# ivanacollg/MPC_CollisionAvoidance

Measured on AMD Instinct MI355X. Metric: batched SQP-RTI solves/sec (USV, N=40 horizon, 10 obstacles), higher is better.
Workload: dtype f64

## Files before the change

mpc_collisionavoidance_amd/csrc/gfx950/lanes.hpp:

```cpp
#pragma once
#include <hip/hip_runtime.h>

#define USV_DEV __device__ __forceinline__

namespace lanes {

constexpr int GROUP = 16;

USV_DEV int lane() { return (int)(threadIdx.x & 15u); }
USV_DEV long group_linear() { return (long)blockIdx.x * (long)(blockDim.x >> 4) + (long)(threadIdx.x >> 4); }

template <int CTRL>
USV_DEV double dpp_mov(double v)
{
    const long l = __builtin_bit_cast(long, v);
    const long r = __builtin_amdgcn_update_dpp(0L, l, CTRL, 0xf, 0xf, true);
    return __builtin_bit_cast(double, r);
}

template <int K>
USV_DEV double bcast(double v)
{
    static_assert(K >= 0 && K < 16, "lane index");
    return dpp_mov<0x150 + K>(v);
// ... 26 lines not shown
}
template <int K0, int K1, int K2>
USV_DEV void fma_bc3(double &c, double b0, double a0, double b1, double a1, double b2, double a2)
{
    asm(USV_DPP_HEAD "v_fmac_f64_dpp %0, %1, %2 row_newbcast:%7 row_mask:0xf bank_mask:0xf\n\t"
        "v_fmac_f64_dpp %0, %3, %4 row_newbcast:%8 row_mask:0xf bank_mask:0xf\n\t"
        "v_fmac_f64_dpp %0, %5, %6 row_newbcast:%9 row_mask:0xf bank_mask:0xf"
        : "+&v"(c) : "v"(b0), "v"(a0), "v"(b1), "v"(a1), "v"(b2), "v"(a2), "n"(K0), "n"(K1), "n"(K2));
}
template <int K0, int K1, int K2, int K3>
USV_DEV void fma_bc4(double &c, double b0, double a0, double b1, double a1, double b2, double a2, double b3, double a3)
{
    asm(USV_DPP_HEAD "v_fmac_f64_dpp %0, %1, %2 row_newbcast:%9 row_mask:0xf bank_mask:0xf\n\t"
        "v_fmac_f64_dpp %0, %3, %4 row_newbcast:%10 row_mask:0xf bank_mask:0xf\n\t"
        "v_fmac_f64_dpp %0, %5, %6 row_newbcast:%11 row_mask:0xf bank_mask:0xf\n\t"
        "v_fmac_f64_dpp %0, %7, %8 row_newbcast:%12 row_mask:0xf bank_mask:0xf"
        : "+&v"(c) : "v"(b0), "v"(a0), "v"(b1), "v"(a1), "v"(b2), "v"(a2), "v"(b3), "v"(a3), "n"(K0), "n"(K1), "n"(K2), "n"(K3));
}

USV_DEV void settle(double &v)
{
    asm volatile("s_nop 1" : "+v"(v));
}

USV_DEV double gather(double v, int src)
{
    const int addr = (int)((((unsigned)threadIdx.x & 48u) | ((unsigned)src & 15u)) << 2);
    const long l = __builtin_bit_cast(long, v);
    const int lo = __builtin_amdgcn_ds_bpermute(addr, (int)l);
    const int hi = __builtin_amdgcn_ds_bpermute(addr, (int)(l >> 32));
    return __builtin_bit_cast(double, ((long)(unsigned)lo) | ((long)hi << 32));
}

template <int N>
USV_DEV double ror(double v)
{
    static_assert(N >= 1 && N < 16, "rotation");
    return dpp_mov<0x120 + N>(v);
}

USV_DEV double gsum(double v)
{
    v += ror<8>(v);
    v += ror<4>(v);
    v += ror<2>(v);
    v += ror<1>(v);
    return v;
}
USV_DEV double vmax(double a, double b)
{
    double r;
    asm("v_max_f64 %0, %1, %2" : "=v"(r) : "v"(a), "v"(b));
    return r;
}
USV_DEV double vmax_abs(double a, double b)
{
    double r;
    asm("v_max_f64 %0, %1, |%2|" : "=v"(r) : "v"(a), "v"(b));
    return r;
}
USV_DEV double vmax_abs2(double a, double b)
{
    double r;
    asm("v_max_f64 %0, |%1|, |%2|" : "=v"(r) : "v"(a), "v"(b));
    return r;
}
USV_DEV double gmax(double v)
{
    v = vmax(v, ror<8>(v));
    v = vmax(v, ror<4>(v));
    v = vmax(v, ror<2>(v));
    v = vmax(v, ror<1>(v));
    return v;
}
USV_DEV double gmin(double v)
{
    v = fmin(v, ror<8>(v));
    v = fmin(v, ror<4>(v));
    v = fmin(v, ror<2>(v));
    v = fmin(v, ror<1>(v));
    return v;
}

USV_DEV int uniform(int v) { return __builtin_amdgcn_readfirstlane(v); }

USV_DEV void sched_fence() { __builtin_amdgcn_sched_barrier(0); }

USV_DEV void count_one(int *p) { atomicAdd(p, 1); }
USV_DEV int fetch_add(int *p) { return atomicAdd(p, 1); }

USV_DEV bool wave_any(bool p) { return __any((int)p) != 0; }

USV_DEV double frcp(double x)
{
    double r = __builtin_amdgcn_rcp(x);
    r = __builtin_fma(__builtin_fma(-x, r, 1.0), r, r);
    r = __builtin_fma(__builtin_fma(-x, r, 1.0), r, r);
    return r;
}
USV_DEV void frcp2(double a, double b, double &ia, double &ib)
{
    const double r = frcp(a * b);
    ia = r * b;
    ib = r * a;
}
USV_DEV double frsqrt(double x)
{
    double y = __builtin_amdgcn_rsq(x);
    y = __builtin_fma(0.5 * y, __builtin_fma(-x * y, y, 1.0), y);
    y = __builtin_fma(0.5 * y, __builtin_fma(-x * y, y, 1.0), y);
    return y;
}

USV_DEV void st_shared(double *p, double v)
{
    __hip_atomic_store(reinterpret_cast<unsigned long long *>(p), __builtin_bit_cast(unsigned long long, v), __ATOMIC_RELAXED, __HIP_MEMORY_SCOPE_AGENT);
}
// ... 119 lines not shown
```

mpc_collisionavoidance_amd/csrc/lin_order.hpp:

```cpp
#pragma once

#if defined(__HIPCC__) || defined(__CUDACC__)
#define USV_HD __host__ __device__ inline
#else
#define USV_HD inline
#endif

namespace usv {

struct LinItem {
    long g;
    int k;
};

USV_HD long lin_slot(long g, long B) { return g < B ? g : B - 1; }

USV_HD LinItem lin_item(long item, int N, long B, const int *perm_cur, const int *inv_next)
{
    const long q = item / (N + 1);
    LinItem it;
    it.k = (int)(item - q * (N + 1));
    it.g = q;
    if (q < B) {
        const long b = perm_cur ? (long)perm_cur[q] : q;
        it.g = inv_next ? (long)inv_next[b] : b;
    }
    return it;
}

}
```

mpc_collisionavoidance_amd/csrc/linearize.hpp:

```cpp
#pragma once
#include "lanes.hpp"
#include "lin_order.hpp"
#include "params.hpp"
#include "sfor.hpp"

namespace usv {

template <class M, class = void>
struct ModelCall {
    struct Pre {};
    USV_DEV static Pre prepare(const double *) { return {}; }
    USV_DEV static void fjvp(const Pre &, const double *x, const double *U, const double *s, const double *su, double *f, double *js)
    {
        M::fjvp(x, U, s, su, f, js);
    }
};
template <class M>
struct ModelCall<M, std::void_t<typename M::Pre>> {
    using Pre = typename M::Pre;
    USV_DEV static Pre prepare(const double *x) { return M::prepare(x); }
    USV_DEV static void fjvp(const Pre &p, const double *x, const double *U, const double *s, const double *su, double *f, double *js)
    {
        M::fjvp_pre(p, x, U, s, su, f, js);
    }
};

template <class M, int KCH, bool SOFT, bool MULTI = false, int MODE = 0>
struct Linearize {
    static constexpr int NX = M::NX, NU = M::NU, NZ = NX + NU;
    using WL = WsLayout<M, KCH, SOFT>;
    static constexpr bool SPEC = MODE == 1 || MODE == 3, FIXUP = MODE == 2 || MODE == 4;

    USV_DEV static void run(const DevPtrs &P, long gid)
    {
        const long Bp = lanes::uniform(P.spec->Bp);
        const int k = (int)(gid / Bp);
        run_at(P, k, gid - (long)k * Bp);
    }

    USV_DEV static void run_item(const DevPtrs &P, long item)
    {
        const LinItem it = lin_item(item, P.spec->N, (long)P.spec->B, P.perm_cur, P.inv_next);
        run_at(P, it.k, it.g);
    }

    USV_DEV static void run_marked(const DevPtrs &P, long g, int row)
    {
        const int N = lanes::uniform(P.spec->N);
        const long gi = lin_slot(g, (long)lanes::uniform(P.spec->B));
        const long b = P.perm ? (long)P.perm[gi] : gi;
        int any = 0;
        for (int w = 0; w < P.redo_words; w++) any |= P.redo[b * P.redo_words + w];
        if (any == 0) return;
        for (int k = row; k <= N; k += lanes::WAVE_ROWS) run_at(P, k, g);
    }

    USV_DEV static void run_at(const DevPtrs &P, const int k, const long g)
    {
// ... 12 lines not shown
            }
        }
        if constexpr (FIXUP) {
            if (((P.redo[b * P.redo_words + (k >> 5)] >> (k & 31)) & 1) == 0) return;
        }
        auto ld = [](const double *q) {
            if constexpr (SPEC) return lanes::ld_shared(q);
            else return *q;
        };
        double *tile = P.ws + (((long)k * Bp + g) * lanes::uniform(S.npt)) * LANES + lane;
        const bool xlane = lane >= NU && lane < NZ;

        double x[NX], U[NU > 0 ? NU : 1];
        const double *xk = P.x + ((long)b * (N + 1) + k) * NX;
        sfor<0, NX>([&](auto i) { x[i] = ld(xk + i); });
        if (k < N) {
            const double *uk = P.u + ((long)b * N + k) * NU;
            sfor<0, NU>([&](auto i) { U[i] = ld(uk + i); });
        } else {
            sfor<0, NU>([&](auto i) { U[i] = 0.0; });
        }

        {
            const double *Mrow = (k < N ? S.Mc : S.Me) + lane * LANES;
            const double *yr = (k < N) ? P.yref + ((long)b * N + k) * S.ny : P.yref_e + (long)b * S.ny_e;
            const int ny = (k < N) ? S.ny : S.ny_e;
            double acc = 0.0;
            for (int y = 0; y < ny; y++) acc = fma(-Mrow[y], yr[y], acc);
            tile[WL::P_GQ * LANES] = acc;
        }
        if (k == N) return;

        const int nsteps = MULTI ? S.sim_steps : 1;
        const double dt = S.dt / (double)nsteps;
        double s0[NX], f[NX], js[NX], xs[NX], ss[NX], xa[NX], sa[NX], su[NU > 0 ? NU : 1];
        sfor<0, NU>([&](auto l) { su[l] = (lane == l) ? 1.0 : 0.0; });
        sfor<0, NX>([&](auto i) { s0[i] = (lane == NU + i) ? 1.0 : 0.0; });
        using MC = ModelCall<M>;
        const typename MC::Pre pre = MC::prepare(x);
        for (int step = 0; step < nsteps; step++) {
            MC::fjvp(pre, x, U, s0, su, f, js);
            sfor<0, NX>([&](auto i) {
                xa[i] = f[i];
                sa[i] = js[i];
                xs[i] = fma(0.5 * dt, f[i], x[i]);
                ss[i] = fma(0.5 * dt, js[i], s0[i]);
            });
            MC::fjvp(pre, xs, U, ss, su, f, js);
            sfor<0, NX>([&](auto i) {
                xa[i] = fma(2.0, f[i], xa[i]);
                sa[i] = fma(2.0, js[i], sa[i]);
                xs[i] = fma(0.5 * dt, f[i], x[i]);
                ss[i] = fma(0.5 * dt, js[i], s0[i]);
            });
            MC::fjvp(pre, xs, U, ss, su, f, js);
            sfor<0, NX>([&](auto i) {
                xa[i] = fma(2.0, f[i], xa[i]);
                sa[i] = fma(2.0, js[i], sa[i]);
                xs[i] = fma(dt, f[i], x[i]);
                ss[i] = fma(dt, js[i], s0[i]);
            });
            MC::fjvp(pre, xs, U, ss, su, f, js);
            sfor<0, NX>([&](auto i) {
                x[i] = fma(dt / 6.0, xa[i] + f[i], x[i]);
                sa[i] = fma(dt / 6.0, sa[i] + js[i], s0[i]);
                if constexpr (MULTI) s0[i] = sa[i];
            });
        }
        const double *xn = P.x + ((long)b * (N + 1) + k + 1) * NX;
        double bres = 0.0;
        sfor<0, NX>([&](auto i) { bres = (lane == NU + i) ? x[i] - ld(xn + i) : bres; });
        using MP = MatPack<M>;
        sfor<0, MP::NPK>([&](auto q) {
            const int sidx = 16 * q + lane;
            double val = 0.0;
            sfor<0, NX>([&](auto j) {
                constexpr int s0 = MP::start(j), cnt = MP::count(j);
                if constexpr (cnt > 0 && s0 < 16 * q + 16 && s0 + cnt > 16 * q) {
                    const int within = sidx - s0;
                    int c_l = 0;
                    sfor<0, cnt>([&](auto ci) { c_l = (within == ci) ? MP::nth(MP::row_mask(j), ci) : c_l; });
                    const double gth = lanes::gather(sa[j], c_l);
                    val = (within >= 0 && within < cnt) ? gth : val;
                }
            });
            tile[(WL::P_MAT + q) * LANES] = val;
        });
        tile[WL::P_RB0 * LANES] = xlane ? bres : 0.0;
    }
};

}
```

mpc_collisionavoidance_amd/csrc/usvmpc.hip:

```cpp
#ifndef USV_PART
#define USV_PART -1
#endif
#define USV_MAIN (USV_PART <= 0)

#include "gfx950/lanes.hpp"

#include "guidance.hpp"
#include "host_spec.hpp"
#include "linearize.hpp"
#include "models.hpp"
#include "obstacle_tracks.hpp"
#include "qp_ipm.hpp"
#include "sim.hpp"
#include "cond_launch.hpp"
#ifdef USV_GEN_MODEL_HEADER
#include USV_GEN_MODEL_HEADER
#endif

#include <algorithm>
#include <cstdint>
#include <cstdio>
#include <cstring>
#include <mutex>
#include <string>
#include <unordered_map>
#include <vector>

using namespace usv;

#ifndef USV_LIN_BLOCKS
#define USV_LIN_BLOCKS 2
#endif
constexpr int LIN_MODES = 5;
constexpr int lin_block(int mode) { return mode == 3 ? 64 : 256; }
template <class M, int KCH, bool SOFT, bool MULTI, int MODE = 0>
__global__ void __launch_bounds__(lin_block(MODE), USV_LIN_BLOCKS) usv_linearize(DevPtrs P, long n)
{
    using L = Linearize<M, KCH, SOFT, MULTI, MODE>;
    if constexpr (MODE == 4) {
        const long g = (long)blockIdx.x * (lin_block(MODE) / 64) + (long)(threadIdx.x >> 6);
        if (g < n) L::run_marked(P, g, (int)lanes::wave_row());
    } else {
        const long gid = lanes::group_linear();
        if (gid >= n) return;
        if constexpr (MODE == 3) L::run_item(P, gid);
        else L::run(P, gid);
    }
}

#ifndef USV_QP_WAVES
#define USV_QP_WAVES 2
#endif
template <int KCH, bool SOFTBOX>
constexpr int qp_waves() { return (KCH >= 2 || SOFTBOX) ? 1 : USV_QP_WAVES; }

template <class M, int KCH, bool SOFT, bool HDIAG, bool PACK, bool SOFTBOX, bool LDSWS = false, bool MERGE = false, bool AUXLDS = false, bool WIDE = false,
          int WW = 1, bool CPC = true>
__global__ void __launch_bounds__(64 * WW, ((LDSWS || WIDE) ? 1 : qp_waves<KCH, SOFTBOX>())) usv_qp_rti(DevPtrs P, long ngroups, int phase, int queue0, int rows)
{
    const int row = (int)(threadIdx.x >> 4);
    const long g0 = (long)blockIdx.x * rows;
    if (g0 >= ngroups) return;
    if constexpr (!WIDE && !LDSWS) { if (P.co_ctl != nullptr && threadIdx.x == 0) lanes::count_one(P.co_ctl + 2); }
    const bool has = row < rows;
    QpIpm<M, KCH, SOFT, HDIAG, PACK, SOFTBOX, LDSWS, MERGE, AUXLDS, WIDE, WW, CPC> q(P, has ? g0 + row : g0, has ? row : -1);
    q.solve(phase, queue0);
}
template <class M, int KCH, bool SOFT, bool MERGE, bool LDSWS = true, int WW = 1, bool SOFTBOX = false, bool UNPACKED = false>
constexpr auto wide_kernel()
{
    if constexpr (SOFTBOX || (UNPACKED && KCH > 0)) {
        if constexpr (WW == 1 && !MERGE) return &usv_qp_rti<M, KCH, SOFT, true, false, SOFTBOX, LDSWS, false, false, true, 1>;
// ... 51 lines not shown
        lanes::acquire_agent();
        {
            QpIpm<M, KCH, SOFT, true, (KCH > 0), false, true, MERGE, false, true, 1> q(P, (long)e, (threadIdx.x >> 4) == 0 ? 0 : -1);
            q.solve(3, -1);
        }
        if (threadIdx.x == 0) lanes::count_one(ctl + 3);
    }
}
static __global__ void usv_co_done(int *ctl) { lanes::publish(ctl + 1, 1); }
using qp_resume_t = void (*)(DevPtrs);
using qp_resume_co_t = void (*)(DevPtrs, int, int, int);
template <class M, int KCH, bool SOFT, bool MERGE, bool LDSWS = false>
constexpr qp_resume_t resume_kernel()
{
    if constexpr (KCH == 1 || (KCH == 0 && !MERGE)) return &usv_qp_resume<M, KCH, SOFT, MERGE, LDSWS>;
    else return nullptr;
}
template <class M, int KCH, bool SOFT, bool MERGE>
constexpr qp_resume_co_t resume_co_kernel()
{
    if constexpr (KCH == 1 || (KCH == 0 && !MERGE)) return &usv_qp_resume_co<M, KCH, SOFT, MERGE>;
    else return nullptr;
}
using qp_kernel_t = void (*)(DevPtrs, long, int, int, int);
using group_kernel_t = void (*)(DevPtrs, long);

struct Kernels {
    qp_kernel_t qp, qp_lds, qp_aux;
    qp_kernel_t wide_lds1, wide_hbm1, wide_lds4, wide_hbm4;
    qp_resume_t resume, resume_lds;
    qp_resume_co_t resume_co;
    int nplw, ex_lds, ex_hbm;
    group_kernel_t lin[2][LIN_MODES];
    group_kernel_t qp_export;
    int npt_hard, npt_soft;
    int kch;
    bool soft;
};

template <class M, int KCH, bool SOFT, bool MERGE, bool SOFTBOX = false, bool UNPACKED = false>
void set_wide(Kernels &k)
{
    using WL = WsLayout<M, KCH, SOFT, SOFTBOX>;
    constexpr bool packed = KCH > 0 && !SOFTBOX && !UNPACKED;
    constexpr bool resumes = !(SOFTBOX || (UNPACKED && KCH > 0));
    k.wide_lds1 = wide_kernel<M, KCH, SOFT, MERGE, true, 1, SOFTBOX, UNPACKED>();
    k.wide_hbm1 = wide_kernel<M, KCH, SOFT, MERGE, false, 1, SOFTBOX, UNPACKED>();
    k.wide_lds4 = wide_kernel<M, KCH, SOFT, MERGE, true, 4, SOFTBOX, UNPACKED>();
    k.wide_hbm4 = wide_kernel<M, KCH, SOFT, MERGE, false, 4, SOFTBOX, UNPACKED>();
    k.resume = resumes ? resume_kernel<M, KCH, SOFT, MERGE>() : nullptr;
    k.resume_lds = resumes ? resume_kernel<M, KCH, SOFT, MERGE, true>() : nullptr;
    k.resume_co = resumes ? resume_co_kernel<M, KCH, SOFT, MERGE>() : nullptr;
    k.nplw = WL::P_RB0 - (packed ? 4 : 0) + (SOFTBOX ? 6 : 0);
    k.ex_lds = wide_ex_planes(KCH, SOFTBOX);
    k.ex_hbm = wide_ex_planes_hbm(KCH, SOFTBOX);
}

template <class M, int KCH, bool SOFT, bool PACK, bool SOFTBOX>
__global__ void __launch_bounds__(64) usv_qp_export(DevPtrs P, long ngroups)
{
    const long g0 = (long)blockIdx.x * 4;
    if (g0 >= ngroups) return;
    QpIpm<M, KCH, SOFT, true, PACK, SOFTBOX> q(P, g0 + (long)(threadIdx.x >> 4));
    q.export_rows();
}

// ... 247 lines not shown
    bool resume_lds, handover_lds;
    long max_waves;
    int ncu;
    long qp_cap;
    bool aux_lds;
    long aux_cap;
    bool map_changed;
    unsigned noise_mask;
    long long instance_offset;
    int *d_fail_ring;
    int *d_unconv_ring;
    unsigned long long *d_unconv_total;
    enum { F_X = 0, F_U, F_STATUS, F_X0, F_YREF, F_YREF_E, F_P, F_LH, F_COUNT };
    char *arena;
    char *mirror;
    size_t arena_bytes, f_off[F_COUNT + 1], f_len[F_COUNT];
    size_t dirty_lo[F_COUNT], dirty_hi[F_COUNT];
    std::vector<char> dirty_stage[F_COUNT];
    bool inflight;
    bool out_valid;
    bool extern_access;
    bool pipeline;
    hipStream_t aux_stream;
    hipEvent_t ev_pre, ev_spec;
    int *d_epoch, *d_redo, *d_perm2, *d_inv;
    long spec_for;
    bool spec_valid;
    bool spec_outstanding;
    int spec_quiet;
    long spec_hits, spec_misses;
    const int *spec_perm;
    bool spec_fine;
    int lin_force;
    int *d_force_epoch, *d_force_redo, *d_force_inv;
    int cond_N2;
    CondDims cond_dims;
    CondDims *d_cond_dims;
    double *d_cond_scratch;
    long cond_teams;
    size_t cond_lds;
    double *d_obs_pos, *d_obs_vel;
    double *d_clear, *d_clear_min;
    bool tracks_on;
    bool tracks_pos_set;
    bool tracks_dirty;
    bool tracks_extern;
    bool step_on_advance;
    bool clear_reset;
    long export_at;
    bool last_cond;
    bool layout_dirty;
    size_t bytes;
    std::string err;
    std::vector<void *> allocs;
};

template <class M, int KCH, bool SOFT>
Kernels kernels_for(const usvmpc_handle *h)
{
    constexpr bool CANPACK = KCH > 0;
    const DevSpec &S = h->spec;
    const bool pack = CANPACK && S.boxpack != 0;
    Kernels k = {};
    k.lin[0][0] = &usv_linearize<M, KCH, SOFT, false, 0>; k.lin[0][1] = &usv_linearize<M, KCH, SOFT, false, 1>; k.lin[0][2] = &usv_linearize<M, KCH, SOFT, false, 2>;
    k.lin[0][3] = &usv_linearize<M, KCH, SOFT, false, 3>; k.lin[0][4] = &usv_linearize<M, KCH, SOFT, false, 4>;
    k.lin[1][0] = &usv_linearize<M, KCH, SOFT, true, 0>; k.lin[1][1] = &usv_linearize<M, KCH, SOFT, true, 1>; k.lin[1][2] = &usv_linearize<M, KCH, SOFT, true, 2>;
    k.lin[1][3] = &usv_linearize<M, KCH, SOFT, true, 3>; k.lin[1][4] = &usv_linearize<M, KCH, SOFT, true, 4>;
    k.qp_export = S.any_bsoft ? &usv_qp_export<M, KCH, SOFT, false, true>
                              : pack ? &usv_qp_export<M, KCH, SOFT, CANPACK, false> : &usv_qp_export<M, KCH, SOFT, false, false>;
    k.npt_hard = WsLayout<M, KCH, SOFT, false>::NPT; k.npt_soft = WsLayout<M, KCH, SOFT, true>::NPT;
    k.kch = KCH; k.soft = SOFT;
    auto qp = [&k](qp_kernel_t q, qp_kernel_t q_lds = nullptr, qp_kernel_t q_aux = nullptr) { k.qp = q; k.qp_lds = q_lds; k.qp_aux = q_aux; };
    const bool merge = pack && h->merge_rows && !S.box_dense;
#ifdef USV_BENCH_ONLY
    if (!(S.hdiag && pack && !S.any_bsoft)) return k;
    if (merge) {
        qp(&usv_qp_rti<M, KCH, SOFT, true, CANPACK, false, false, CANPACK>, &usv_qp_rti<M, KCH, SOFT, true, CANPACK, false, true, CANPACK>,
           &usv_qp_rti<M, KCH, SOFT, true, CANPACK, false, false, CANPACK, true>);
        set_wide<M, KCH, SOFT, CANPACK>(k);
    } else {
        qp(&usv_qp_rti<M, KCH, SOFT, true, CANPACK, false>, &usv_qp_rti<M, KCH, SOFT, true, CANPACK, false, true>,
           &usv_qp_rti<M, KCH, SOFT, true, CANPACK, false, false, false, true>);
    }
#else
    if (S.any_bsoft) {
        if (S.hdiag) { qp(&usv_qp_rti<M, KCH, SOFT, true, false, true>); set_wide<M, KCH, SOFT, false, true>(k); }
        else qp(&usv_qp_rti<M, KCH, SOFT, false, false, true>);
    } else if (S.hdiag) {
        if (merge) {
            qp(&usv_qp_rti<M, KCH, SOFT, true, CANPACK, false, false, CANPACK>, &usv_qp_rti<M, KCH, SOFT, true, CANPACK, false, true, CANPACK>,
               &usv_qp_rti<M, KCH, SOFT, true, CANPACK, false, false, CANPACK, true>);
            set_wide<M, KCH, SOFT, CANPACK>(k);
        } else if (pack) {
            qp(&usv_qp_rti<M, KCH, SOFT, true, CANPACK, false>, &usv_qp_rti<M, KCH, SOFT, true, CANPACK, false, true>,
               &usv_qp_rti<M, KCH, SOFT, true, CANPACK, false, false, false, true>);
            set_wide<M, KCH, SOFT, false>(k);
        } else {
            qp(&usv_qp_rti<M, KCH, SOFT, true, false, false>, &usv_qp_rti<M, KCH, SOFT, true, false, false, true>);
            set_wide<M, KCH, SOFT, false, false, true>(k);
        }
// ... 598 lines not shown
        HIP_TRY(h, hipMemsetAsync(h->d_susp_list, 0xff, (size_t)h->B * sizeof(int), h->stream));
        HIP_TRY(h, hipEventRecord(h->ev_co_pre, h->stream));
    }
    hipLaunchKernelGGL(kern, qg, qb, aux_bytes, h->stream, h->ptrs, ng, phase, q0, 4);
    if (co) {
        hipLaunchKernelGGL(usv_co_done, dim3(1), dim3(1), 0, h->stream, h->ptrs.co_ctl);
        HIP_TRY(h, hipStreamWaitEvent(h->co_stream, h->ev_co_pre, 0));
        long nco = std::min<long>(h->resume_cap, (long)h->B);
        nco = std::min<long>(nco, h->co_wgs > 0 ? (long)h->co_wgs : (long)std::max(h->ncu, 1));
        hipLaunchKernelGGL(k.resume_co, dim3((unsigned)nco), dim3(qp_block), xbytes, h->co_stream, h->ptrs, (int)qg.x, (int)h->B, h->co_spin_limit);
        HIP_TRY(h, hipEventRecord(h->ev_co_end, h->co_stream));
    }
    if (hand) {
        HIP_TRY(h, hipEventRecord(ev[3], h->stream));
        h->ev3_set[h->nsolves % usvmpc_handle::RING] = true;
        const long nwg = std::min<long>(h->resume_cap, (long)h->B);
        hipLaunchKernelGGL(kern_resume, dim3((unsigned)nwg), dim3(qp_block), xbytes, h->stream, h->ptrs);
    }
    if (co) HIP_TRY(h, hipStreamWaitEvent(h->stream, h->ev_co_end, 0));
    return 0;
}

int launch_solve(usvmpc_handle *h, const Kernels &k, int phase)
{
    {
        const int rcf = mirror_flush(h);
        if (rcf) return rcf;
    }
    if (h->tracks_on && (h->tracks_dirty || h->tracks_extern)) {
        const int rct = tracks_predict(h);
        if (rct) return rct;
    }
    const long lin_groups = (long)(h->N + 1) * h->Bp;
    auto lin_count = [&](int mode) { return mode == 4 ? (long)h->Bp : lin_groups; };
    auto lin_grid = [&](int mode) {
        const long per_block = mode == 4 ? lin_block(mode) / 64 : lin_block(mode) / LANES;
        return dim3((unsigned)((lin_count(mode) + per_block - 1) / per_block));
    };
    hipEvent_t *ev = h->ev[h->nsolves % usvmpc_handle::RING];
    const int B = h->B;
    auto sort_into = [&](int *dst, int *inv) {
        const int *prev2 = h->sort_two ? h->d_iter_prev : h->ptrs.qp_iter;
        hipLaunchKernelGGL(usv_sort_hist, dim3((B + 255) / 256), dim3(256), 0, h->stream, h->ptrs.qp_iter, prev2, B, h->d_hist);
        hipLaunchKernelGGL(usv_sort_scan, dim3(1), dim3(64), 0, h->stream, h->d_hist, h->d_cursor);
        hipLaunchKernelGGL(usv_sort_scatter, dim3((B + 255) / 256), dim3(256), 0, h->stream, h->ptrs.qp_iter, prev2, B, h->d_cursor, dst, inv);
    };
    const group_kernel_t *lin = k.lin[h->spec.sim_steps > 1 ? 1 : 0];
    const bool cond = phase == 0 && h->cond_N2 > 0;
    const bool pipe = phase == 0 && h->pipeline && !h->mirror && !h->extern_access && h->dynamic_rows && h->B >= 16384 && !cond;
    if (pipe && !h->aux_stream) {
        int prio_least = 0, prio_greatest = 0;
        HIP_TRY(h, hipDeviceGetStreamPriorityRange(&prio_least, &prio_greatest));
        HIP_TRY(h, hipStreamCreateWithPriority(&h->aux_stream, hipStreamNonBlocking, prio_least));
        HIP_TRY(h, hipEventCreateWithFlags(&h->ev_pre, hipEventDisableTiming));
        HIP_TRY(h, hipEventCreateWithFlags(&h->ev_spec, hipEventDisableTiming));
        if (dev_alloc(h, &h->d_epoch, (size_t)B, false) || dev_alloc(h, &h->d_redo, (size_t)B * ((h->N + 32) / 32), true) ||
            dev_alloc(h, &h->d_perm2, (size_t)B, true) || dev_alloc(h, &h->d_inv, (size_t)B, true))
            return USVMPC_E_HIP;
        HIP_TRY(h, hipMemsetAsync(h->d_epoch, 0xff, (size_t)B * sizeof(int), h->stream));
    }
    if (h->spec_outstanding) {
        HIP_TRY(h, hipStreamWaitEvent(h->stream, h->ev_spec, 0));
        h->spec_outstanding = false;
    }
    const bool had_spec = pipe && h->spec_for == h->nsolves;
    const bool use_spec = had_spec && h->spec_valid;
    if (had_spec) (use_spec ? h->spec_hits : h->spec_misses)++;
    h->spec_valid = false;
    if (use_spec) {
        h->ptrs.perm = h->spec_perm;
        h->map_changed = true;
    } else if (h->sort_enabled && h->nsolves > 0 && phase != 2) {
        if (phase == 0) h->map_changed = true;
        sort_into(h->d_perm, nullptr);
        HIP_TRY(h, hipGetLastError());
        h->ptrs.perm = h->d_perm;
    }
    constexpr int SPEC_QUIET_MIN = 2;
    if (pipe) h->spec_quiet++;
    const bool spec_next = pipe && h->spec_quiet >= SPEC_QUIET_MIN;
// ... 265 lines not shown
#ifdef USV_GEN_ONLY
    if (d->model != USVMPC_MODEL_GENERATED) {
        std::fprintf(stderr, "usvmpc_create: this library only holds the generated model\n");
        return USVMPC_E_ARG;
    }
#endif
    int ndev = 0;
    if (hipGetDeviceCount(&ndev) != hipSuccess || ndev < 1 || d->device < 0 || d->device >= ndev) {
        std::fprintf(stderr, "usvmpc_create: no usable HIP device (count %d, requested %d); there is no CPU fallback\n",
                     ndev, d->device);
        return USVMPC_E_NODEVICE;
    }
    usvmpc_handle *h = new usvmpc_handle();
    h->desc = *d;
    h->spec = S;
    model_dims(d->model, h->nx, h->nu);
    h->nz = h->nx + h->nu; h->ny = S.ny; h->ny_e = S.ny_e;
    h->N = S.N; h->K = S.K; h->B = S.B; h->Bp = S.Bp;
    h->kch = d->model == USVMPC_MODEL_USV ? 0 : ((S.K + LANES - 1) / LANES > 1 ? 2 : 1);
    h->soft = d->soft != 0 || d->model == USVMPC_MODEL_GUIDANCE_CA1;
#ifdef USV_GEN_MODEL_HEADER
    if (d->model == USVMPC_MODEL_GENERATED) { h->kch = USV_GEN_KCH; h->soft = USV_GEN_SOFT != 0; }
#endif
    h->device = d->device;
    h->bytes = 0; h->nsolves = 0; h->own_stream = true;
    h->map_changed = false;
    h->export_at = -1;
    h->layout_dirty = false;
    h->last_cond = false;
    h->pipeline = true;
    h->aux_stream = nullptr; h->ev_pre = nullptr; h->ev_spec = nullptr;
    h->d_epoch = nullptr; h->d_redo = nullptr; h->d_perm2 = nullptr; h->d_inv = nullptr;
    h->spec_fine = false;
    h->lin_force = 0; h->d_force_epoch = nullptr; h->d_force_redo = nullptr; h->d_force_inv = nullptr;
    h->spec_for = -1; h->spec_valid = false; h->spec_outstanding = false; h->spec_perm = nullptr;
    h->spec_quiet = 0; h->spec_hits = 0; h->spec_misses = 0;
    h->noise_mask = ~0u;
    h->instance_offset = 0;
    h->d_obs_pos = nullptr; h->d_obs_vel = nullptr; h->d_clear = nullptr; h->d_clear_min = nullptr;
    h->tracks_on = false; h->tracks_pos_set = false; h->tracks_dirty = false; h->tracks_extern = false;
    h->step_on_advance = true; h->clear_reset = false;
    h->cond_N2 = 0; h->d_cond_dims = nullptr; h->d_cond_scratch = nullptr; h->cond_teams = 0; h->cond_lds = 0;
    h->dynamic_rows = true;
    h->qp_cap = 0;
    h->aux_lds = true;
    h->aux_cap = 0;
    h->lds_mode = -1;
    h->lds_cap = 0;
    h->wide_mode = -1; h->wide_cap = 0; h->wide_hbm_cap = 0; h->last_wide = 0;
    h->wide_waves = -1; h->wide4_cap = 0; h->wide4_hbm_cap = 0;
    h->handover_co = -1; h->co_spin_limit = 200000; h->co_wgs = 0; h->co_ready = false; h->co_stream = nullptr; h->ev_co_pre = nullptr; h->ev_co_end = nullptr; h->d_co_ctl = nullptr;
    h->handover_iter = -1; for (bool &e : h->ev3_set) e = false; h->resume_lds = false; h->handover_lds = true; h->d_susp_count = nullptr; h->d_susp_list = nullptr; h->d_susp_rec = nullptr; h->resume_cap = 0;
    h->max_waves = 0;
    {
        hipDeviceProp_t prop;
        h->ncu = (hipGetDeviceProperties(&prop, d->device) == hipSuccess) ? prop.multiProcessorCount : 0;
    }
    std::memset(&h->ptrs, 0, sizeof(h->ptrs));
    auto fail = [&](int rc) {
        std::fprintf(stderr, "usvmpc_create: %s\n", h->err.c_str());
        for (void *a : h->allocs) (void)hipFree(a);
        if (h->mirror) (void)hipHostFree(h->mirror);
        delete h;
        return rc;
    };
#define TRY_C(x) do { int rc_ = (x); if (rc_) return fail(rc_); } while (0)
// ... 513 lines not shown
        return 0;
    }
    if (s == "max_waves") { h->max_waves = (long)value; reset_caps(h); cond_release(h); return 0; }
    if (s == "keep_multipliers") {
        if (value == 0.0) return 0;
        DevPtrs &P = h->ptrs;
        if (!P.lam_out) {
            HIP_TRY(h, hipSetDevice(h->device));
            P.nlam = lam_len(h->spec, h->soft);
            const size_t cnt = (size_t)h->B * (h->N + 1) * (size_t)(P.nlam > 0 ? P.nlam : 1);
            if (dev_alloc(h, &P.lam_out, cnt, false)) return USVMPC_E_HIP;
            if (dev_alloc(h, &P.t_out, cnt, false)) { P.lam_out = nullptr; return USVMPC_E_HIP; }
            h->export_at = -1;
        }
        return 0;
    }
    if (s == "qp_cond_N") {
        const int n2 = (int)value;
        if (n2 < 0 || n2 > h->N) { h->err = "qp_cond_N must lie in 0..N"; return USVMPC_E_ARG; }
        const int want = (n2 == 0 || n2 == h->N) ? 0 : n2;
        if (want > 0) {
            if (h->nx + ((h->N + want - 1) / want) * h->nu > 64) { h->err = "qp_cond_N: a condensed stage may have at most 64 variables (nx + ceil(N / qp_cond_N) nu)"; return USVMPC_E_ARG; }
            if (h->spec.any_bsoft) { h->err = "partial condensing (qp_cond_N) is not built for soft state bounds"; return USVMPC_E_ARG; }
        }
        if (want != h->cond_N2) { cond_release(h); h->cond_N2 = want; h->map_changed = true; }
        return 0;
    }
    if (s == "sort_two_ticks") { h->sort_two = value != 0.0; return 0; }
    if (s == "lin_force_modes") {
        if (value != 0.0 && value != 1.0 && value != 2.0) { h->err = "lin_force_modes: 0, 1 or 2"; return USVMPC_E_ARG; }
        h->lin_force = (int)value;
        return 0;
    }
    if (s == "aux_in_lds") { h->aux_lds = value != 0.0; reset_caps(h); return 0; }
    if (s == "lds_workspace") {
        h->lds_mode = value < 0.0 ? -1 : (value > 0.0 ? 1 : 0);
        reset_caps(h);
        return 0;
    }
    if (s == "wide") {
        h->wide_mode = value < 0.0 ? -1 : (value > 0.0 ? 1 : 0);
        reset_caps(h);
        return 0;
    }
    if (s == "wide_waves") {
        h->wide_waves = value < 0.0 ? -1 : (value >= 4.0 ? 4 : 1);
        reset_caps(h);
        return 0;
    }
    if (s == "dynamic_rows") {
        h->dynamic_rows = value != 0.0;
        reset_caps(h);
        return 0;
    }
    if (s == "cond_pred_corr" || s == "cpc_factor" || s == "hpipm_mode") {
        if (s == "cpc_factor") { if (!(value > 0.0)) { h->err = "cpc_factor must be positive"; return USVMPC_E_ARG; } h->spec.cpc_factor = value; }
        else if (s == "hpipm_mode") {
            usvmpc_desc d;
            if (value != (double)(int)value || !hpipm_profile(d, (int)value)) { h->err = "hpipm_mode must be one of USVMPC_HPIPM_*"; return USVMPC_E_ARG; }
            h->spec.mu0 = d.mu0; h->spec.alpha_min = d.alpha_min; h->spec.cpc = d.cond_pred_corr; h->spec.cpc_factor = d.cpc_factor;
        } else {
            h->spec.cpc = value != 0.0 ? 1 : 0;
        }
        HIP_TRY(h, hipSetDevice(h->device));
        HIP_TRY(h, hipMemcpyAsync(h->d_spec, &h->spec, sizeof(DevSpec), hipMemcpyHostToDevice, h->stream));
        HIP_TRY(h, hipStreamSynchronize(h->stream));
// ... 401 lines not shown
```

Baseline: 1.011 million.

## Pack several linearization items per wave using only nonzero Jacobian columns

Adds a packed linearize kernel in which each 64-lane wave integrates several (stage, instance) items at once. Each lane carries only one sensitivity direction whose Jacobian column is structurally nonzero, instead of a full 16-lane group per item. Results are then scattered into the 16-lane workspace tiles through cross-lane bpermute gathers over several store rounds. It is on by default for the multi-step RK4 path when the column mask allows more than four items per wave. This is meant to cut wasted lanes in the RK4 VDE integration, in exchange for extra gather traffic, a serial store loop and higher register pressure.

```diff
diff --git a/mpc_collisionavoidance_amd/csrc/gfx950/lanes.hpp b/mpc_collisionavoidance_amd/csrc/gfx950/lanes.hpp
--- a/mpc_collisionavoidance_amd/csrc/gfx950/lanes.hpp
+++ b/mpc_collisionavoidance_amd/csrc/gfx950/lanes.hpp
@@ -82,6 +82,16 @@
     return __builtin_bit_cast(double, ((long)(unsigned)lo) | ((long)hi << 32));
 }
 
+USV_DEV double gather_wave(double v, int src)
+{
+    const int addr = (int)(((unsigned)src & 63u) << 2);
+    const long l = __builtin_bit_cast(long, v);
+    const int lo = __builtin_amdgcn_ds_bpermute(addr, (int)l);
+    const int hi = __builtin_amdgcn_ds_bpermute(addr, (int)(l >> 32));
+    return __builtin_bit_cast(double, ((long)(unsigned)lo) | ((long)hi << 32));
+}
+USV_DEV int gather_wave_i(int v, int src) { return __builtin_amdgcn_ds_bpermute((int)(((unsigned)src & 63u) << 2), v); }
+
 template <int N>
 USV_DEV double ror(double v)
 {
@@ -133,6 +143,10 @@
 }
 
 USV_DEV int uniform(int v) { return __builtin_amdgcn_readfirstlane(v); }
+
+USV_DEV void park(int &v) { asm volatile("" : "+v"(v)); }
+template <class T>
+USV_DEV void park(T *&p) { asm volatile("" : "+v"(p)); }
 
 USV_DEV void sched_fence() { __builtin_amdgcn_sched_barrier(0); }
 
diff --git a/mpc_collisionavoidance_amd/csrc/lin_order.hpp b/mpc_collisionavoidance_amd/csrc/lin_order.hpp
--- a/mpc_collisionavoidance_amd/csrc/lin_order.hpp
+++ b/mpc_collisionavoidance_amd/csrc/lin_order.hpp
@@ -15,11 +15,10 @@
 
 USV_HD long lin_slot(long g, long B) { return g < B ? g : B - 1; }
 
-USV_HD LinItem lin_item(long item, int N, long B, const int *perm_cur, const int *inv_next)
+USV_HD LinItem lin_item_at(long q, int k, long B, const int *perm_cur, const int *inv_next)
 {
-    const long q = item / (N + 1);
     LinItem it;
-    it.k = (int)(item - q * (N + 1));
+    it.k = k;
     it.g = q;
     if (q < B) {
         const long b = perm_cur ? (long)perm_cur[q] : q;
@@ -28,4 +27,10 @@
     return it;
 }
 
+USV_HD LinItem lin_item(long item, int N, long B, const int *perm_cur, const int *inv_next)
+{
+    const long q = item / (N + 1);
+    return lin_item_at(q, (int)(item - q * (N + 1)), B, perm_cur, inv_next);
 }
+
+}
diff --git a/mpc_collisionavoidance_amd/csrc/lin_pack.hpp b/mpc_collisionavoidance_amd/csrc/lin_pack.hpp
--- /dev/null
+++ b/mpc_collisionavoidance_amd/csrc/lin_pack.hpp
@@ -0,0 +1,66 @@
+#pragma once
+#include "lin_order.hpp"
+
+namespace usv {
+
+constexpr int LIN_PACK_WAVE = 64, LIN_PACK_ROWS = 4;
+
+USV_HD constexpr int lin_pack_popcount(unsigned m)
+{
+    int n = 0;
+    for (; m != 0u; m &= m - 1u) n++;
+    return n;
+}
+USV_HD constexpr int lin_pack_nth(unsigned mask, int i)
+{
+    for (int b = 0; b < 32; b++)
+        if ((mask >> b) & 1u) {
+            if (i == 0) return b;
+            i--;
+        }
+    return 0;
+}
+USV_HD constexpr int lin_pack_rank(unsigned mask, int b) { return lin_pack_popcount(mask & ((1u << b) - 1u)); }
+
+USV_HD constexpr int lin_pack_nc(unsigned cm) { return lin_pack_popcount(cm); }
+USV_HD constexpr int lin_pack_ipw(unsigned cm) { return cm != 0u ? LIN_PACK_WAVE / lin_pack_nc(cm) : 0; }
+USV_HD constexpr int lin_pack_rounds(unsigned cm) { return (lin_pack_ipw(cm) + LIN_PACK_ROWS - 1) / LIN_PACK_ROWS; }
+USV_HD constexpr bool lin_pack_pays(unsigned cm) { return lin_pack_ipw(cm) > LIN_PACK_ROWS; }
+USV_HD constexpr long lin_pack_waves(unsigned cm, long n) { return (n + lin_pack_ipw(cm) - 1) / lin_pack_ipw(cm); }
+
+struct LinPackLane {
+    int slot;
+    int col;
+    bool on;
+};
+USV_HD constexpr LinPackLane lin_pack_lane(unsigned cm, int l)
+{
+    const int nc = lin_pack_nc(cm), ipw = lin_pack_ipw(cm);
+    int slot = l / nc;
+    const int rk = l - slot * nc;
+    const bool on = slot < ipw;
+    slot = on ? slot : ipw - 1;
+    int col = 0;
+    for (int i = 0; i < nc; i++) col = (rk == i) ? lin_pack_nth(cm, i) : col;
+    return LinPackLane{slot, col, on};
+}
+USV_HD constexpr int lin_pack_base(unsigned cm, int slot) { return slot * lin_pack_nc(cm); }
+USV_HD constexpr int lin_pack_src(unsigned cm, int slot, int c) { return lin_pack_base(cm, slot) + lin_pack_rank(cm, c); }
+
+USV_HD constexpr int lin_pack_store_slot(int round, int row) { return LIN_PACK_ROWS * round + row; }
+USV_HD constexpr bool lin_pack_store_on(unsigned cm, int round, int row, long nitems)
+{
+    return lin_pack_store_slot(round, row) < lin_pack_ipw(cm) && (long)lin_pack_store_slot(round, row) < nitems;
+}
+
+struct LinPackSplit {
+    long q;
+    int r;
+};
+USV_HD constexpr LinPackSplit lin_pack_split(long q0, int r0, int slot, int period)
+{
+    const unsigned t = (unsigned)r0 + (unsigned)slot, d = t / (unsigned)period;
+    return LinPackSplit{q0 + (long)d, (int)(t - d * (unsigned)period)};
+}
+
+}
diff --git a/mpc_collisionavoidance_amd/csrc/linearize.hpp b/mpc_collisionavoidance_amd/csrc/linearize.hpp
--- a/mpc_collisionavoidance_amd/csrc/linearize.hpp
+++ b/mpc_collisionavoidance_amd/csrc/linearize.hpp
@@ -24,6 +24,44 @@
         M::fjvp_pre(p, x, U, s, su, f, js);
     }
 };
+
+template <class M, bool MULTI>
+USV_DEV void erk4_vde(const typename ModelCall<M>::Pre &pre, double *x, const double *U, double *s0, const double *su, const double dt,
+                      const int nsteps, double *sa)
+{
+    constexpr int NX = M::NX;
+    using MC = ModelCall<M>;
+    double f[NX], js[NX], xs[NX], ss[NX], xa[NX];
+    for (int step = 0; step < nsteps; step++) {
+        MC::fjvp(pre, x, U, s0, su, f, js);
+        sfor<0, NX>([&](auto i) {
+            xa[i] = f[i];
+            sa[i] = js[i];
+            xs[i] = fma(0.5 * dt, f[i], x[i]);
+            ss[i] = fma(0.5 * dt, js[i], s0[i]);
+        });
+        MC::fjvp(pre, xs, U, ss, su, f, js);
+        sfor<0, NX>([&](auto i) {
+            xa[i] = fma(2.0, f[i], xa[i]);
+            sa[i] = fma(2.0, js[i], sa[i]);
+            xs[i] = fma(0.5 * dt, f[i], x[i]);
+            ss[i] = fma(0.5 * dt, js[i], s0[i]);
+        });
+        MC::fjvp(pre, xs, U, ss, su, f, js);
+        sfor<0, NX>([&](auto i) {
+            xa[i] = fma(2.0, f[i], xa[i]);
+            sa[i] = fma(2.0, js[i], sa[i]);
+            xs[i] = fma(dt, f[i], x[i]);
+            ss[i] = fma(dt, js[i], s0[i]);
+        });
+        MC::fjvp(pre, xs, U, ss, su, f, js);
+        sfor<0, NX>([&](auto i) {
+            x[i] = fma(dt / 6.0, xa[i] + f[i], x[i]);
+            sa[i] = fma(dt / 6.0, sa[i] + js[i], s0[i]);
+            if constexpr (MULTI) s0[i] = sa[i];
+        });
+    }
+}
 
 template <class M, int KCH, bool SOFT, bool MULTI = false, int MODE = 0>
 struct Linearize {
@@ -102,41 +140,11 @@
         if (k == N) return;
 
         const int nsteps = MULTI ? S.sim_steps : 1;
-        const double dt = S.dt / (double)nsteps;
-        double s0[NX], f[NX], js[NX], xs[NX], ss[NX], xa[NX], sa[NX], su[NU > 0 ? NU : 1];
+        double s0[NX], sa[NX], su[NU > 0 ? NU : 1];
         sfor<0, NU>([&](auto l) { su[l] = (lane == l) ? 1.0 : 0.0; });
         sfor<0, NX>([&](auto i) { s0[i] = (lane == NU + i) ? 1.0 : 0.0; });
-        using MC = ModelCall<M>;
-        const typename MC::Pre pre = MC::prepare(x);
-        for (int step = 0; step < nsteps; step++) {
-            MC::fjvp(pre, x, U, s0, su, f, js);
-            sfor<0, NX>([&](auto i) {
-                xa[i] = f[i];
-                sa[i] = js[i];
-                xs[i] = fma(0.5 * dt, f[i], x[i]);
-                ss[i] = fma(0.5 * dt, js[i], s0[i]);
-            });
-            MC::fjvp(pre, xs, U, ss, su, f, js);
-            sfor<0, NX>([&](auto i) {
-                xa[i] = fma(2.0, f[i], xa[i]);
-                sa[i] = fma(2.0, js[i], sa[i]);
-                xs[i] = fma(0.5 * dt, f[i], x[i]);
-                ss[i] = fma(0.5 * dt, js[i], s0[i]);
-            });
-            MC::fjvp(pre, xs, U, ss, su, f, js);
-            sfor<0, NX>([&](auto i) {
-                xa[i] = fma(2.0, f[i], xa[i]);
-                sa[i] = fma(2.0, js[i], sa[i]);
-                xs[i] = fma(dt, f[i], x[i]);
-                ss[i] = fma(dt, js[i], s0[i]);
-            });
-            MC::fjvp(pre, xs, U, ss, su, f, js);
-            sfor<0, NX>([&](auto i) {
-                x[i] = fma(dt / 6.0, xa[i] + f[i], x[i]);
-                sa[i] = fma(dt / 6.0, sa[i] + js[i], s0[i]);
-                if constexpr (MULTI) s0[i] = sa[i];
-            });
-        }
+        const typename ModelCall<M>::Pre pre = ModelCall<M>::prepare(x);
+        erk4_vde<M, MULTI>(pre, x, U, s0, su, S.dt / (double)nsteps, nsteps, sa);
         const double *xn = P.x + ((long)b * (N + 1) + k + 1) * NX;
         double bres = 0.0;
         sfor<0, NX>([&](auto i) { bres = (lane == NU + i) ? x[i] - ld(xn + i) : bres; });
diff --git a/mpc_collisionavoidance_amd/csrc/linearize_packed.hpp b/mpc_collisionavoidance_amd/csrc/linearize_packed.hpp
--- /dev/null
+++ b/mpc_collisionavoidance_amd/csrc/linearize_packed.hpp
@@ -0,0 +1,137 @@
+#pragma once
+#include "lin_pack.hpp"
+#include "linearize.hpp"
+
+namespace usv {
+
+template <class M, int KCH, bool SOFT, bool MULTI = true, int MODE = 0>
+struct LinearizePacked {
+    static_assert(MODE == 0 || MODE == 1 || MODE == 3, "the fix-up modes keep the 16-lane form");
+    static_assert(MULTI, "the packed form is bit-identical by construction only where the seeds are carried through the step loop");
+    static constexpr int NX = M::NX, NU = M::NU, NZ = NX + NU;
+    using WL = WsLayout<M, KCH, SOFT>;
+    using MP = MatPack<M>;
+    static constexpr unsigned CM = MP::col_mask();
+    static constexpr int NC = lin_pack_nc(CM), IPW = lin_pack_ipw(CM), ROUNDS = lin_pack_rounds(CM);
+    static constexpr bool PAYS = lin_pack_pays(CM);
+    static constexpr bool SPEC = MODE == 1 || MODE == 3, ORDERED = MODE == 3;
+
+    USV_DEV static long uniform_div(long item, int period, long n)
+    {
+        if (n <= 0x7fffffffL) return (long)((unsigned)item / (unsigned)period);
+        return item / period;
+    }
+
+    USV_DEV static void run(const DevPtrs &P, const long item0, const long n)
+    {
+        const DevSpec &S = *P.spec;
+        const int wl = (int)lanes::wave_lane();
+        const int N = lanes::uniform(S.N), Bp = lanes::uniform(S.Bp), B = lanes::uniform(S.B);
+        auto ld = [](const double *q) {
+            if constexpr (SPEC) return lanes::ld_shared(q);
+            else return *q;
+        };
+
+        const LinPackLane me = lin_pack_lane(CM, wl);
+        const bool item_on = item0 + me.slot < n;
+        const int period = ORDERED ? N + 1 : Bp;
+        const long q0 = uniform_div(item0, period, n);
+        const LinPackSplit sp = lin_pack_split(q0, (int)(item0 - q0 * period), item_on ? me.slot : 0, period);
+        int k, g;
+        if constexpr (ORDERED) {
+            const LinItem it = lin_item_at(sp.q, sp.r, (long)B, P.perm_cur, P.inv_next);
+            k = it.k;
+            g = (int)it.g;
+        } else {
+            k = (int)sp.q;
+            g = sp.r;
+        }
+        const long gi = lin_slot((long)g, (long)B);
+        const int b = P.perm ? P.perm[gi] : (int)gi;
+        int ready = 1;
+        if constexpr (SPEC) {
+            const long owner = P.perm_cur ? (long)P.perm_cur[gi] : gi;
+            ready = (lanes::observe(P.epoch + b) == P.tick && lanes::observe(P.epoch + owner) == P.tick) ? 1 : 0;
+            if (ready == 0 && me.on && item_on && wl == lin_pack_base(CM, me.slot)) lanes::set_bits(P.redo + (long)b * P.redo_words + (k >> 5), 1 << (k & 31));
+            if (!lanes::wave_any(ready != 0)) return;
+        }
+        const bool term = k >= N;
+
+        double x[NX], U[NU > 0 ? NU : 1];
+        const double *xk = P.x + ((long)b * (N + 1) + k) * NX;
+        sfor<0, NX>([&](auto i) { x[i] = ld(xk + i); });
+        const double *uk = P.u + ((long)b * N + (term ? N - 1 : k)) * NU;
+        sfor<0, NU>([&](auto i) { U[i] = ld(uk + i); });
+
+        int N_park = N, Bp_park = Bp, ny_park = S.ny, nye_park = S.ny_e;
+        lanes::park(N_park);
+        lanes::park(Bp_park);
+        lanes::park(ny_park);
+        lanes::park(nye_park);
+        int npt_park = S.npt;
+        lanes::park(npt_park);
+        const double *x_park = P.x, *Mc_park = S.Mc, *Me_park = S.Me;
+        lanes::park(x_park);
+        lanes::park(Mc_park);
+        lanes::park(Me_park);
+
+        int col = me.col;
+        lanes::park(col);
+        col &= 15;
+        const int nsteps = MULTI ? S.sim_steps : 1;
+        double s0[NX], sa[NX], su[NU > 0 ? NU : 1];
+        sfor<0, NU>([&](auto l) { su[l] = (col == l) ? 1.0 : 0.0; });
+        sfor<0, NX>([&](auto i) { s0[i] = (col == NU + i) ? 1.0 : 0.0; });
+        const typename ModelCall<M>::Pre pre = ModelCall<M>::prepare(x);
+        erk4_vde<M, MULTI>(pre, x, U, s0, su, S.dt / (double)nsteps, nsteps, sa);
+
+        const int row = wl >> 4, lane = wl & 15;
+        const int N2 = lanes::uniform(N_park), Bp2 = lanes::uniform(Bp_park), ny_c = lanes::uniform(ny_park), ny_e = lanes::uniform(nye_park);
+        const int npt = lanes::uniform(npt_park);
+        const bool xlane = lane >= NU && lane < NZ;
+#pragma unroll 1
+        for (int r = 0; r < ROUNDS; r++) {
+            const int slot = lin_pack_store_slot(r, row);
+            const bool on = lin_pack_store_on(CM, r, row, n - item0);
+            const int base = lin_pack_base(CM, on ? slot : 0);
+            const int k2 = lanes::gather_wave_i(k, base), g2 = lanes::gather_wave_i(g, base), b2 = lanes::gather_wave_i(b, base);
+            const bool live = on && lanes::gather_wave_i(ready, base) != 0;
+            double *tile = P.ws + (((long)k2 * Bp2 + g2) * npt) * LANES + lane;
+
+            {
+                const double *Mrow = (k2 < N2 ? Mc_park : Me_park) + lane * LANES;
+                const double *yr = (k2 < N2) ? P.yref + ((long)b2 * N2 + k2) * ny_c : P.yref_e + (long)b2 * ny_e;
+                const int ny = (k2 < N2) ? ny_c : ny_e;
+                double acc = 0.0;
+                for (int y = 0; y < ny; y++) acc = fma(-Mrow[y], yr[y], acc);
+                if (live) tile[WL::P_GQ * LANES] = acc;
+            }
+            const bool dyn = live && k2 < N2;
+            sfor<0, MP::NPK>([&](auto q) {
+                const int sidx = 16 * q + lane;
+                double val = 0.0;
+                sfor<0, NX>([&](auto j) {
+                    constexpr int st = MP::start(j), cnt = MP::count(j);
+                    if constexpr (cnt > 0 && st < 16 * q + 16 && st + cnt > 16 * q) {
+                        const int within = sidx - st;
+                        int c_r = 0;
+                        sfor<0, cnt>([&](auto ci) { c_r = (within == ci) ? lin_pack_rank(CM, MP::nth(MP::row_mask(j), ci)) : c_r; });
+                        const double gth = lanes::gather_wave(sa[j], base + c_r);
+                        val = (within >= 0 && within < cnt) ? gth : val;
+                    }
+                });
+                if (dyn) tile[(WL::P_MAT + q) * LANES] = val;
+            });
+            const int xi_own = xlane ? lane - NU : 0;
+            const double xn_own = ld(x_park + ((long)b2 * (N2 + 1) + (k2 < N2 ? k2 + 1 : k2)) * NX + xi_own);
+            double bres = 0.0;
+            sfor<0, NX>([&](auto i) {
+                const double xi = lanes::gather_wave(x[i], base);
+                bres = (lane == NU + i) ? xi - xn_own : bres;
+            });
+            if (dyn) tile[WL::P_RB0 * LANES] = xlane ? bres : 0.0;
+        }
+    }
+};
+
+}
diff --git a/mpc_collisionavoidance_amd/csrc/usvmpc.hip b/mpc_collisionavoidance_amd/csrc/usvmpc.hip
--- a/mpc_collisionavoidance_amd/csrc/usvmpc.hip
+++ b/mpc_collisionavoidance_amd/csrc/usvmpc.hip
@@ -8,6 +8,7 @@
 #include "guidance.hpp"
 #include "host_spec.hpp"
 #include "linearize.hpp"
+#include "linearize_packed.hpp"
 #include "models.hpp"
 #include "obstacle_tracks.hpp"
 #include "qp_ipm.hpp"
@@ -33,11 +34,17 @@
 #endif
 constexpr int LIN_MODES = 5;
 constexpr int lin_block(int mode) { return mode == 3 ? 64 : 256; }
-template <class M, int KCH, bool SOFT, bool MULTI, int MODE = 0>
+template <class M, int KCH, bool SOFT, bool MULTI, bool PACKED, int MODE = 0>
 __global__ void __launch_bounds__(lin_block(MODE), USV_LIN_BLOCKS) usv_linearize(DevPtrs P, long n)
 {
     using L = Linearize<M, KCH, SOFT, MULTI, MODE>;
-    if constexpr (MODE == 4) {
+    if constexpr (PACKED) {
+        using LP = LinearizePacked<M, KCH, SOFT, MULTI, MODE>;
+        const long wave = (long)lanes::uniform((int)(blockIdx.x * (unsigned)(lin_block(MODE) / 64) + (threadIdx.x >> 6)));
+        const long item0 = wave * LP::IPW;
+        if (item0 >= n) return;
+        LP::run(P, item0, n);
+    } else if constexpr (MODE == 4) {
         const long g = (long)blockIdx.x * (lin_block(MODE) / 64) + (long)(threadIdx.x >> 6);
         if (g < n) L::run_marked(P, g, (int)lanes::wave_row());
     } else {
@@ -155,6 +162,8 @@
     qp_resume_co_t resume_co;
     int nplw, ex_lds, ex_hbm;
     group_kernel_t lin[2][LIN_MODES];
+    group_kernel_t lin_packed[2][LIN_MODES];
+    int lin_ipw;
     group_kernel_t qp_export;
     int npt_hard, npt_soft;
     int kch;
@@ -468,6 +477,7 @@
     const int *spec_perm;
     bool spec_fine;
     int lin_force;
+    bool lin_packed;
     int *d_force_epoch, *d_force_redo, *d_force_inv;
     int cond_N2;
     CondDims cond_dims;
@@ -498,10 +508,17 @@
     const DevSpec &S = h->spec;
     const bool pack = CANPACK && S.boxpack != 0;
     Kernels k = {};
-    k.lin[0][0] = &usv_linearize<M, KCH, SOFT, false, 0>; k.lin[0][1] = &usv_linearize<M, KCH, SOFT, false, 1>; k.lin[0][2] = &usv_linearize<M, KCH, SOFT, false, 2>;
-    k.lin[0][3] = &usv_linearize<M, KCH, SOFT, false, 3>; k.lin[0][4] = &usv_linearize<M, KCH, SOFT, false, 4>;
-    k.lin[1][0] = &usv_linearize<M, KCH, SOFT, true, 0>; k.lin[1][1] = &usv_linearize<M, KCH, SOFT, true, 1>; k.lin[1][2] = &usv_linearize<M, KCH, SOFT, true, 2>;
-    k.lin[1][3] = &usv_linearize<M, KCH, SOFT, true, 3>; k.lin[1][4] = &usv_linearize<M, KCH, SOFT, true, 4>;
+    k.lin[0][0] = &usv_linearize<M, KCH, SOFT, false, false, 0>; k.lin[0][1] = &usv_linearize<M, KCH, SOFT, false, false, 1>;
+    k.lin[0][2] = &usv_linearize<M, KCH, SOFT, false, false, 2>; k.lin[0][3] = &usv_linearize<M, KCH, SOFT, false, false, 3>;
+    k.lin[0][4] = &usv_linearize<M, KCH, SOFT, false, false, 4>;
+    k.lin[1][0] = &usv_linearize<M, KCH, SOFT, true, false, 0>; k.lin[1][1] = &usv_linearize<M, KCH, SOFT, true, false, 1>;
+    k.lin[1][2] = &usv_linearize<M, KCH, SOFT, true, false, 2>; k.lin[1][3] = &usv_linearize<M, KCH, SOFT, true, false, 3>;
+    k.lin[1][4] = &usv_linearize<M, KCH, SOFT, true, false, 4>;
+    if constexpr (lin_pack_pays(MatPack<M>::col_mask())) {
+        k.lin_ipw = lin_pack_ipw(MatPack<M>::col_mask());
+        k.lin_packed[1][0] = &usv_linearize<M, KCH, SOFT, true, true, 0>; k.lin_packed[1][1] = &usv_linearize<M, KCH, SOFT, true, true, 1>;
+        k.lin_packed[1][3] = &usv_linearize<M, KCH, SOFT, true, true, 3>;
+    }
     k.qp_export = S.any_bsoft ? &usv_qp_export<M, KCH, SOFT, false, true>
                               : pack ? &usv_qp_export<M, KCH, SOFT, CANPACK, false> : &usv_qp_export<M, KCH, SOFT, false, false>;
     k.npt_hard = WsLayout<M, KCH, SOFT, false>::NPT; k.npt_soft = WsLayout<M, KCH, SOFT, true>::NPT;
@@ -1166,9 +1183,12 @@
         if (rct) return rct;
     }
     const long lin_groups = (long)(h->N + 1) * h->Bp;
+    const group_kernel_t *lin16 = k.lin[h->spec.sim_steps > 1 ? 1 : 0], *linp = k.lin_packed[h->spec.sim_steps > 1 ? 1 : 0];
+    auto lin_is_packed = [&](int mode) { return h->lin_packed && k.lin_ipw > 0 && linp[mode] != nullptr; };
     auto lin_count = [&](int mode) { return mode == 4 ? (long)h->Bp : lin_groups; };
     auto lin_grid = [&](int mode) {
-        const long per_block = mode == 4 ? lin_block(mode) / 64 : lin_block(mode) / LANES;
+        const long waves_per_block = lin_block(mode) / 64;
+        const long per_block = lin_is_packed(mode) ? waves_per_block * k.lin_ipw : mode == 4 ? waves_per_block : lin_block(mode) / LANES;
         return dim3((unsigned)((lin_count(mode) + per_block - 1) / per_block));
     };
     hipEvent_t *ev = h->ev[h->nsolves % usvmpc_handle::RING];
@@ -1179,7 +1199,8 @@
         hipLaunchKernelGGL(usv_sort_scan, dim3(1), dim3(64), 0, h->stream, h->d_hist, h->d_cursor);
         hipLaunchKernelGGL(usv_sort_scatter, dim3((B + 255) / 256), dim3(256), 0, h->stream, h->ptrs.qp_iter, prev2, B, h->d_cursor, dst, inv);
     };
-    const group_kernel_t *lin = k.lin[h->spec.sim_steps > 1 ? 1 : 0];
+    const group_kernel_t lin[LIN_MODES] = {lin_is_packed(0) ? linp[0] : lin16[0], lin_is_packed(1) ? linp[1] : lin16[1], lin16[2],
+                                           lin_is_packed(3) ? linp[3] : lin16[3], lin16[4]};
     const bool cond = phase == 0 && h->cond_N2 > 0;
     const bool pipe = phase == 0 && h->pipeline && !h->mirror && !h->extern_access && h->dynamic_rows && h->B >= 16384 && !cond;
     if (pipe && !h->aux_stream) {
@@ -1511,6 +1532,7 @@
     h->aux_stream = nullptr; h->ev_pre = nullptr; h->ev_spec = nullptr;
     h->d_epoch = nullptr; h->d_redo = nullptr; h->d_perm2 = nullptr; h->d_inv = nullptr;
     h->spec_fine = false;
+    h->lin_packed = true;
     h->lin_force = 0; h->d_force_epoch = nullptr; h->d_force_redo = nullptr; h->d_force_inv = nullptr;
     h->spec_for = -1; h->spec_valid = false; h->spec_outstanding = false; h->spec_perm = nullptr;
     h->spec_quiet = 0; h->spec_hits = 0; h->spec_misses = 0;
@@ -2090,6 +2112,7 @@
         h->lin_force = (int)value;
         return 0;
     }
+    if (s == "lin_packed") { h->lin_packed = value != 0.0; return 0; }
     if (s == "aux_in_lds") { h->aux_lds = value != 0.0; reset_caps(h); return 0; }
     if (s == "lds_workspace") {
         h->lds_mode = value < 0.0 ? -1 : (value > 0.0 ? 1 : 0);
```

Result: slower. 860,200 (-14.9%).
